# mkangquantum/quits

Hardware: AMD Instinct MI355X
Metric: decoded shots/sec + logical-error-rate, [[144,12,12]] BB code, d rounds, p=0.003 (higher is better)
Workload: dtype f32

## Files before the change

### quits_amd/csrc/bp_scatter_wide.hip

```cpp
#include "qd_internal.h"
#include "../../include/quits_amd.h"
#include "bp_scatter_edge.h"

#ifndef QSW_SCAT_SGPR_POS
#define QSW_SCAT_SGPR_POS 1
#endif
#ifndef QSW_GPRIO
#define QSW_GPRIO 1
#endif
#ifndef QSW_FAST_START
#define QSW_FAST_START 1
#endif
#ifndef QSW_THIN_LAST
#define QSW_THIN_LAST 1
#endif
#ifndef QSW_PRIO_BASE
#define QSW_PRIO_BASE 0
#endif

__device__ __forceinline__ uint4 qs_reuse4(uint4 &v) { asm volatile("" : "+v"(v.x), "+v"(v.y), "+v"(v.z), "+v"(v.w)); return v; }

template <int T, int MW, int CPL, int NSW>
__global__ void __launch_bounds__(T, MW) qd_bp_scatter_wide_kernel(BpGraphDev g, ScatGraphDev sg, DecodeArgs a, ScatArgs x)
{
// ... 310 lines not shown
            }
            return;
        }
    }
    for (int b = tid; b < sg.nslots; b += T)
        if (*QS_LDS(cur + 4u * (uint32_t)b) < 0) {
            const uint32_t jf = sg.slot_fault[b];
            if (jf != 0xFFFFFFFFu) atomicOr(&outw[jf >> 5], 1u << (jf & 31u));
        }
    if (!converged && a.want_llr && tid == 0) misc[48] = atomicAdd(a.fail_count, 1);
    __syncthreads();
    for (int w = tid; w < g.out_words; w += T) a.err_bits[shot * g.out_words + w] = outw[w];
    if (!converged && a.want_llr) {
        const int slot = misc[48];
        float *dst = a.llr_ws + (int64_t)slot * n_pad;
        for (int k1 = tid; k1 < g.n; k1 += T) dst[k1] = (float)(*QS_LDS(cur + 4u * sg.k1_slot[k1]) + 1) * x.grid_inv;
        if (tid == 0) a.fail_list[slot] = (int32_t)shot;
    }
    if (tid == 0) a.status[shot] = t | (converged << 16) | a.status_or;
}

#undef QS_ACC
#define QS_ACC(off) (prior_g[((uint32_t)(off) - (uint32_t)sg.offA) >> 2])
#define QS_ADJ(row_) qs_as_uint4(__builtin_amdgcn_raw_buffer_load_b128(adj_rsrc, adj_voff, (row_) * adj_row, 0))
#define QS_ABL_ADJC
template <int NSW>
__global__ void __launch_bounds__(64) qd_bp_first_pass_kernel(BpGraphDev g, ScatGraphDev sg, const int32_t *prior_g, uint32_t *rec)
{
    static_assert(NSW == 3, "the record has room for three sign words");
    const int c = (int)blockIdx.x * 64 + (int)threadIdx.x;
    const bool actv = c < g.m;
    constexpr int j = 0;
// ... 59 lines not shown
```

### quits_amd/csrc/osd_shared.h

```cpp
#pragma once
#include "qd_internal.h"

#define QD_NOKEY 0xFFFFFFFFu

#ifdef QD_OSD_TIMING
#define QD_TICK(slot)                                                                   \
    {                                                                                   \
        const unsigned long long now_ = wall_clock64();                                 \
        acc_[slot] += now_ - tick_;                                                     \
        tick_ = now_;                                                                   \
    }
#else
#define QD_TICK(slot)
#endif

__device__ __forceinline__ uint64_t &qd_qword(uint64_t *q_lds, uint64_t *q_glb, int kw_lds, int m_pad, int w, int r)
{
    return (w < kw_lds) ? q_lds[(size_t)w * m_pad + r] : q_glb[(size_t)(w - kw_lds) * m_pad + r];
}

__device__ __forceinline__ uint32_t qd_mono_key(float llr)
{
    const float f = llr + 0.0f;
    const uint32_t u = __float_as_uint(f);
    return (u & 0x80000000u) ? ~u : (u | 0x80000000u);
}

template <int T>
__device__ __forceinline__ void qd_bitonic_u64(uint64_t *buf, int P, int tid)
{
    for (int k = 2; k <= P; k <<= 1)
        for (int j = k >> 1; j > 0; j >>= 1) {
            for (int pi = tid; pi < (P >> 1); pi += T) {
                const int i = ((pi & ~(j - 1)) << 1) | (pi & (j - 1));
                const int l = i | j;
                const uint64_t x = buf[i], y = buf[l];
                const bool up = ((i & k) == 0);
                if ((x > y) == up) { buf[i] = y; buf[l] = x; }
            }
            __syncthreads();
        }
}

#define QD_OSD_TIER 1024
#ifndef QD_OSD_FULL_PAIRS
#define QD_OSD_FULL_PAIRS 1
#endif
#ifndef QD_OSD_TIER_FIRST
#define QD_OSD_TIER_FIRST 256
#endif
#define QD_OSD_KWR 6
#ifndef QD_OSD_KWR0
#define QD_OSD_KWR0 2
#endif
#ifndef QD_OSD_KPT
#define QD_OSD_KPT 1
#endif

template <int T>
__device__ __forceinline__ uint32_t qd_block_sum(uint32_t v, uint32_t *buf, int &phase)
{
    constexpr int NW = T / 64;
    v = qd_wave_add(v);
    if ((threadIdx.x & 63) == 0) buf[phase * 64 + (threadIdx.x >> 6)] = v;
// ... 19 lines not shown
    const uint8_t *det, *upd;
    int64_t det_stride, det_offset, upd_stride;
    const float *llr_ws;
    const int32_t *fail_list, *fail_count;
    const int32_t *slot_list, *slot_count;
    uint64_t *q_spill_fast;
    uint64_t *mt_ws;
    uint32_t *err_bits;
    int32_t *status;
    unsigned long long *dbg;
};

struct TierState {
    uint32_t lo_key, lo_idx; int sphase, exhausted, limit;
    uint32_t guess = 0u, cut = 0u, count = 0u;
};

#ifndef QD_OSD_TIER_INLINE
#define QD_OSD_TIER_INLINE __forceinline__
#endif
template <int T, int KPT = QD_OSD_KPT, class ARGS = OsdRegArgs, int SCAN = 0>
__device__ QD_OSD_TIER_INLINE int qd_osd_draw_tier(const ARGS &a, const float *llr, uint64_t *sortbuf, uint16_t *order,
                                             uint32_t *red, uint32_t *sumbuf, TierState &ts)
{
    const int tid = threadIdx.x;
    const int n = a.n;
    const bool in_regs = n <= KPT * T;
    uint32_t lo_key = ts.lo_key, lo_idx = ts.lo_idx;
    int sphase = ts.sphase;
    const uint32_t lim = (uint32_t)ts.limit;
    bool exhausted = false;
    int cnt = 0;
    {
            uint32_t kreg[KPT];
            if (in_regs) {
#pragma unroll
                for (int i = 0; i < KPT; ++i) {
                    const int b = tid + i * T;
                    kreg[i] = (b < n) ? qd_mono_key(llr[b]) : 0xFFFFFFFFu;
                }
            }
            auto scan_keys = [&](auto fn) {
                if constexpr (SCAN == 0) {
                    for (int b = tid; b < n; b += T) fn(qd_mono_key(llr[b]), b);
                } else {
                    const float4 *l4 = reinterpret_cast<const float4 *>(llr);
                    const int n4 = n >> 2;
                    for (int b0 = 0; b0 < n4; b0 += SCAN * T) {
// ... 137 lines not shown
                if (take) {
                    const uint32_t at = atomicAdd(&red[80], 1u);
                    if (at < (uint32_t)QD_OSD_TIER) sortbuf[at] = ((uint64_t)u << 32) | j;
                }
            });
            __syncthreads();
            if (!spec) break;
            {
                const uint32_t c = (uint32_t)__builtin_amdgcn_readfirstlane((int)red[80]);
                ts.count = c;
                if (c > 0u && c <= lim) { cnt = (int)c; lo_key = t_hi; ts.cut = t_hi; break; }
                spec = false;
                __syncthreads();
            }
            }
            int P = 64;
            while (P < cnt) P <<= 1;
            for (int i = cnt + tid; i < P; i += T) sortbuf[i] = ~0ull;
            __syncthreads();
            if (cnt <= 256 && cnt <= T) {
                if ((tid & ~63) < cnt) {
                    const uint64_t mine = tid < cnt ? sortbuf[tid] : ~0ull;
                    const uint4 *sb4 = reinterpret_cast<const uint4 *>(sortbuf);
                    int rank = 0;
                    for (int i = 0; i < (cnt + 1) / 2; ++i) {
                        const uint4 v = sb4[i];
                        const uint64_t k0 = (uint64_t)v.x | ((uint64_t)v.y << 32), k1 = (uint64_t)v.z | ((uint64_t)v.w << 32);
                        rank += (k0 < mine ? 1 : 0) + (k1 < mine ? 1 : 0);
                    }
                    if (tid < cnt) order[rank] = (uint16_t)(mine & 0xFFFFu);
                }
            } else {
                qd_bitonic_u64<T>(sortbuf, P, tid);
                for (int i = tid; i < cnt; i += T) order[i] = (uint16_t)(sortbuf[i] & 0xFFFFu);
            }
            __syncthreads();
    }
    ts.lo_key = lo_key; ts.lo_idx = lo_idx; ts.sphase = sphase; ts.exhausted = 0;
    return cnt;
}

struct OsdLds {
    uint64_t *q;
    uint64_t *tb;
    uint8_t *sp;
    int16_t *rowpiv;
    uint16_t *prow;
    uint32_t *pcol;
    uint32_t *pairs;
    uint32_t *bcols;
    uint32_t *red;
    uint32_t *outw;
// ... 177 lines not shown
```

### quits_amd/csrc/osd_sr.hip

```cpp
#include "osd_shared.h"
#include <algorithm>

#ifndef QD_SR_TIER_GUESS
#define QD_SR_TIER_GUESS 1
#endif
struct OsdSrArgs {
    int m, n, m_pad, n_pad, mw, out_words, upd_rows, ell_log2;
    int o_tb, o_rowpiv, o_prow, o_pcol, o_ppos, o_nz, o_cand, o_stq, o_stsp, o_bcols, o_red, o_out, o_order;
    int tier_first;
    const uint16_t *csc_ell;
    const uint32_t *bit_orig;
    const uint8_t *det, *upd;
    int64_t det_stride, det_offset, upd_stride;
    const float *llr_ws;
    const int32_t *fail_list, *fail_count;
    uint64_t *q_spill;
    int32_t *hard_list, *hard_count;
    uint32_t *err_bits;
    int32_t *status;
    unsigned long long *dbg;
};

template <int T, int RPT, int KWR>
__global__ void __launch_bounds__(T, QD_SR_WPS_OF(RPT)) qd_osd0_sr_kernel(OsdSrArgs a)
{
    extern __shared__ __align__(16) unsigned char smem[];
#if QD_SR_PRIO
    __builtin_amdgcn_s_setprio(QD_SR_PRIO);
#endif
    const int tid = threadIdx.x, lane = tid & 63;
    constexpr int NW = T / 64;
    static_assert(NW <= 16 && T >= 256, "key / flag records hold 16 wavefronts; the tier drawing wants >= 256 threads");
    uint64_t *tb = reinterpret_cast<uint64_t *>(smem + a.o_tb);
    uint64_t *sortbuf = tb;
    int16_t *rowpiv = reinterpret_cast<int16_t *>(smem + a.o_rowpiv);
    uint16_t *prow = reinterpret_cast<uint16_t *>(smem + a.o_prow);
    uint32_t *pcol = reinterpret_cast<uint32_t *>(smem + a.o_pcol);
    uint16_t *ppos = reinterpret_cast<uint16_t *>(smem + a.o_ppos);
    uint64_t *nz = reinterpret_cast<uint64_t *>(smem + a.o_nz);
    uint32_t *cand = reinterpret_cast<uint32_t *>(smem + a.o_cand);
    uint64_t *stq = reinterpret_cast<uint64_t *>(smem + a.o_stq);
    uint32_t *stsp = reinterpret_cast<uint32_t *>(smem + a.o_stsp);
    uint32_t *bcols = reinterpret_cast<uint32_t *>(smem + a.o_bcols);
    uint32_t *red = reinterpret_cast<uint32_t *>(smem + a.o_red);
    uint32_t *sumbuf = red + 96;
    uint32_t *outw = reinterpret_cast<uint32_t *>(smem + a.o_out);
    uint16_t *order = reinterpret_cast<uint16_t *>(smem + a.o_order);
    const int m = a.m, m_pad = a.m_pad, mw = a.mw, dlog = a.ell_log2;
    uint64_t *qglb = a.q_spill + (size_t)blockIdx.x * (size_t)(mw > KWR ? mw - KWR : 0) * m_pad;
    const int nfail = *a.fail_count;
    if (tid == 0) red[81] = 0u;
    for (int item = blockIdx.x; item < nfail; item += gridDim.x) {
        const int slot = item;
        const int64_t shot = a.fail_list[slot];
        const float *llr = a.llr_ws + (int64_t)slot * a.n_pad;
        const uint8_t *det = a.det + shot * a.det_stride + a.det_offset;
        const uint8_t *upd = a.upd ? a.upd + shot * a.upd_stride : nullptr;
#ifdef QD_OSD_TIMING
        unsigned long long acc_[12] = {0, 0, 0, 0, 0, 0, 0, 0, 0, 0, 0, 0};
        unsigned long long tick_ = wall_clock64();
#endif
        uint64_t my_tb[RPT], my_q[RPT][KWR];
        uint32_t my_sp = 0, my_piv = 0;
#pragma unroll
        for (int i = 0; i < RPT; ++i) {
            const int r = tid + i * T;
            uint32_t sbit = 0;
            if (r < m) {
                sbit = det[r] & 1u;
                if (upd && r < a.upd_rows) sbit ^= upd[r] & 1u;
            }
            my_sp |= sbit << i;
            my_tb[i] = 0ull;
#pragma unroll
            for (int w = 0; w < KWR; ++w) my_q[i][w] = 0ull;
            if (r < m_pad) rowpiv[r] = -1;
        }
        for (int w = tid; w < a.out_words; w += T) outw[w] = 0u;
        if (tid < 240) cand[tid] = (tid % 80) < 64 ? QD_NOKEY : 0u;
        if (tid == 0) red[72] = 0u;
        __syncthreads();
        QD_TICK(10)

        int npiv = 0, done = 0, draining = 0, cmaxp1 = 64, sphase = 0, rd = 0, bseq = 0, ntier = 0;
        uint32_t my_bp = 0;
        uint32_t lo_key = 0, lo_idx = 0;
        while (!done) {
            TierState ts{lo_key, lo_idx, sphase, 0, ntier == 0 ? a.tier_first : QD_OSD_TIER};
            const bool first_tier = ntier == 0;
            if (first_tier) ts.guess = red[81];
            ++ntier;
            const int cnt = qd_osd_draw_tier<T, QD_OSD_KPT, OsdSrArgs, 6>(a, llr, sortbuf, order, red, sumbuf, ts);
            lo_key = ts.lo_key; lo_idx = ts.lo_idx; sphase = ts.sphase;
            if (first_tier && QD_SR_TIER_GUESS) {
                const uint32_t lim1 = (uint32_t)a.tier_first, step = 1u << 20;
                uint32_t g = ts.guess;
                if (ts.cut) g = ts.count * 20u > lim1 * 17u ? ts.cut - step : (ts.count * 20u < lim1 * 11u ? ts.cut + step : ts.cut);
                else if (g) g = ts.count > lim1 ? g - step : g;
                if (g > 0xFFFFFFFFu - step) g = 0u;
                if (tid == 0) red[81] = g;
            }
            QD_TICK(0)
            if (ts.exhausted) break;
            for (int base = 0; base < cnt && !done; base += 64, ++bseq) {
                const int nb = min(64, cnt - base);
#pragma unroll
                for (int i = 0; i < RPT; ++i) { const int r = tid + i * T; if (r < m_pad) tb[r] = 0ull; }
                if (tid < mw) nz[tid] = 0ull;
                if (tid < 64) bcols[tid] = tid < nb ? (uint32_t)order[base + tid] : 0xFFFFFFFFu;
                __syncthreads();
                for (int x = tid; x < (64 << dlog); x += T) {
                    const int c = x >> dlog, q = x & ((1 << dlog) - 1);
                    const uint32_t col = bcols[c];
                    if (col != 0xFFFFFFFFu) {
                        const uint32_t r = a.csc_ell[((size_t)col << dlog) + q];
// ... 173 lines not shown
            if (draining && ((my_bp >> i) & 1u) && (int)(ppos[rowpiv[r]] & 63u) >= cmaxp1) ++over;
        }
        const uint32_t tot = qd_block_sum<T>(over | (resid << 16), sumbuf, sphase);
        const int inconsistent = (tot >> 16) != 0u;
        const int npiv_rep = npiv - (int)(tot & 0xFFFFu);
        if (inconsistent) {
            if (tid == 0) a.hard_list[atomicAdd(a.hard_count, 1)] = slot;
        } else {
#pragma unroll
            for (int i = 0; i < RPT; ++i)
                if (((my_piv >> i) & 1u) && ((my_sp >> i) & 1u)) {
                    const uint32_t j = pcol[rowpiv[tid + i * T]];
                    atomicOr(&outw[j >> 5], 1u << (j & 31u));
                }
            __syncthreads();
            for (int w = tid; w < a.out_words; w += T) a.err_bits[shot * a.out_words + w] = outw[w];
            if (tid == 0) a.status[shot] = (a.status[shot] & 0xFFFF) | (1 << 17) | (min(npiv_rep, 4095) << 20);
        }
        QD_TICK(3)
#ifdef QD_OSD_TIMING
        if (tid == 0) {
            for (int i = 0; i < 8; ++i) atomicAdd(&a.dbg[i], acc_[i]);
            atomicAdd(&a.dbg[8], 1ull); atomicAdd(&a.dbg[9], (unsigned long long)npiv); atomicAdd(&a.dbg[10], acc_[10]); atomicAdd(&a.dbg[11], acc_[11]); atomicAdd(&a.dbg[12], (unsigned long long)ntier); atomicAdd(&a.dbg[13], (unsigned long long)bseq);
        }
#endif
        __syncthreads();
    }
}

int qd_osd_sr_layout(int m, int m_pad, int n, int out_words, int *off13, int *threads, int *rpt)
{
    if (m > 2048 || n > 49152) return 0;
    const int T = m <= 256 ? 256 : (m <= 4 * QD_SR_TSMALL ? QD_SR_TSMALL : 512);
    *threads = T; *rpt = (m + T - 1) / T;
    auto al = [](int x) { return (x + 15) & ~15; };
    int o = 0;
    off13[0] = o; o += al(std::max(m_pad * 8, QD_OSD_TIER * 8));
    off13[1] = o; o += al(m_pad * 2);
    off13[2] = o; o += al(m_pad * 2);
    off13[3] = o; o += al(m_pad * 4);
    off13[4] = o; o += al(m_pad * 2);
    off13[5] = o; o += al(((m + 63) / 64) * 8);
    off13[6] = o; o += 3 * 80 * 4;
    off13[7] = o; o += (QD_SR_KWR_MAX + 1) * 64 * 8;
    off13[8] = o; o += 64 * 4;
    off13[9] = o; o += 64 * 4;
    off13[10] = o; o += 1024;
    off13[11] = o; o += al(out_words * 4);
    off13[12] = o; o += al(QD_OSD_TIER * 2);
    return o;
}

size_t qd_osd_sr_ws_words(int m_pad, int mw, int threads, int rpt)
{
    (void)threads;
    const int kwr = QD_SR_KWR_OF(rpt);
    return (size_t)(mw > kwr ? mw - kwr : 0) * m_pad + 64;
}

hipError_t qd_launch_osd0_sr(const OsdGraphDev &g, const BpGraphDev &bg, const DecodeArgs &a, int blocks, hipStream_t s)
{
    OsdSrArgs r{};
    r.m = g.m; r.n = g.n; r.m_pad = g.m_pad; r.n_pad = bg.n_pad; r.mw = g.mw; r.out_words = bg.out_words; r.upd_rows = a.upd_rows;
    r.ell_log2 = g.ell_log2;
    const int *o = g.s_off;
    r.o_tb = o[0]; r.o_rowpiv = o[1]; r.o_prow = o[2]; r.o_pcol = o[3]; r.o_ppos = o[4]; r.o_nz = o[5]; r.o_cand = o[6]; r.o_stq = o[7];
    r.o_stsp = o[8]; r.o_bcols = o[9]; r.o_red = o[10]; r.o_out = o[11]; r.o_order = o[12];
    r.tier_first = QD_OSD_TIER_FIRST;
    r.csc_ell = g.csc_ell; r.bit_orig = bg.bit_orig;
    r.det = a.det; r.upd = a.upd; r.det_stride = a.det_stride; r.det_offset = a.det_offset; r.upd_stride = a.upd_stride;
    r.llr_ws = a.llr_ws; r.fail_list = a.fail_list; r.fail_count = a.fail_count; r.q_spill = a.q_spill_sr;
    r.hard_list = a.hard_list; r.hard_count = a.hard_count;
    r.err_bits = a.err_bits; r.status = a.status; r.dbg = a.dbg;
    const int lds = g.s_lds_bytes;
#define QD_SR_CASE(TT, RR)                                                                                                        \
    {                                                                                                                             \
        auto k = qd_osd0_sr_kernel<TT, RR, QD_SR_KWR_OF(RR)>;                                                                            \
        hipError_t e = hipFuncSetAttribute((const void *)k, hipFuncAttributeMaxDynamicSharedMemorySize, lds);                     \
        if (e != hipSuccess) return e;                                                                                            \
        hipLaunchKernelGGL(k, dim3((unsigned)blocks), dim3(TT), lds, s, r);                                                       \
        return hipGetLastError();                                                                                                 \
    }
    if (g.s_threads == 256) {
        switch (g.s_rpt) {
        case 1: QD_SR_CASE(256, 1)
        case 2: QD_SR_CASE(256, 2)
        case 3: QD_SR_CASE(256, 3)
        default: QD_SR_CASE(256, 4)
// ... 11 lines not shown
```

### quits_amd/csrc/qd_api.hip

```cpp
#include "../../include/quits_amd.h"
#include "qd_internal.h"

#include <algorithm>
#include <cmath>
#include <cstdarg>
#include <cstdio>
#include <cstdlib>
#include <cstring>
#include <memory>
#include <numeric>
#include <vector>

#define QD_GEN_PREFIX_LDS (32 * 1024)

hipError_t qd_launch_bp(const BpGraphDev &g, const DecodeArgs &a, int64_t B, hipStream_t s);
hipError_t qd_launch_bp_scatter(const BpGraphDev &g, const ScatGraphDev &sg, const DecodeArgs &a, const ScatArgs &x, int64_t B, hipStream_t s);
hipError_t qd_launch_bp_scatter_wide(const BpGraphDev &g, const ScatGraphDev &sg, const DecodeArgs &a, const ScatArgs &x, int64_t B, hipStream_t s);
hipError_t qd_launch_bp_first_pass(const BpGraphDev &g, const ScatGraphDev &sg, const int32_t *prior_g, uint32_t *rec, hipStream_t s);
hipError_t qd_launch_bp_general(const GenGraphDev &g, const BpGraphDev &bg, const DecodeArgs &a, const GenWs &w, int bp_method,
                                int schedule, int64_t shot0, int nshots, hipStream_t s, GenStagePlan *plan);
hipError_t qd_launch_hold(const int32_t *count, int threshold, int microseconds, hipStream_t s);
int qd_bp_ps_lds_bytes(const GenGraphDev &g, int max_rdeg);
hipError_t qd_launch_bp_ps_lds(const GenGraphDev &g, const BpGraphDev &bg, const DecodeArgs &a, int64_t B, hipStream_t s);
hipError_t qd_launch_osd0(const OsdGraphDev &g, const BpGraphDev &bg, const DecodeArgs &a, int blocks_fast,
// ... 49 lines not shown
        size_t bytes = std::max<size_t>(h.size() * sizeof(Tp), 16);
        if (hipMalloc(&d, bytes) != hipSuccess) return -1;
        ptrs.push_back(d);
        if (!h.empty() && hipMemcpy(d, h.data(), h.size() * sizeof(Tp), hipMemcpyHostToDevice) != hipSuccess) return -1;
        *out = reinterpret_cast<const Tp *>(d);
        return 0;
    }
    void release()
    {
        for (void *p : ptrs) (void)hipFree(p);
        ptrs.clear();
    }
};

struct Switches {
    bool no_scatter, scatter_cpl1, scatter_wide_t704, scatter_natural_rounds, scatter_banks_by_slot, scatter_walk_greedy, osdcs_old, bp_no_fast_start;
    float scatter_m2_limit;
    std::vector<int> gen_stages;
};

static Switches read_switches()
{
    auto env = [](const char *name) { return std::getenv(name); };
    Switches w{};
    w.no_scatter = env("QD_NO_SCATTER") != nullptr;
    w.scatter_cpl1 = env("QD_SCATTER_CPL1") != nullptr;
    w.scatter_wide_t704 = env("QD_SCATTER_WIDE_T704") != nullptr;
    w.scatter_natural_rounds = env("QD_SCATTER_NATURAL_ROUNDS") != nullptr;
    w.scatter_banks_by_slot = env("QD_SCATTER_BANKS_BY_SLOT") != nullptr;
    w.scatter_walk_greedy = env("QD_SCATTER_WALK_GREEDY") != nullptr;
    const char *ev = env("QD_BP_NO_FAST_START");
    w.bp_no_fast_start = ev && std::atoi(ev) == 1;
    ev = env("QD_OSDCS_OLD");
    w.osdcs_old = ev && std::atoi(ev) == 1;
    ev = env("QD_SCATTER_M2_LIMIT");
    w.scatter_m2_limit = ev ? (float)std::atof(ev) : INFINITY;
    w.gen_stages = {3, 6, 10, 14, 20, 28, 40, 56, 80, 112};
    if ((ev = env("QD_GEN_STAGES"))) {
        w.gen_stages.clear();
        for (const char *q = ev; *q;) {
            char *end = nullptr;
            const long v = std::strtol(q, &end, 10);
            if (end == q) break;
            if (v > 0) w.gen_stages.push_back((int)v);
            q = *end ? end + 1 : end;
        }
    }
// ... 63 lines not shown
    GenStagePlan gsp{};
    int gen_bounds[QD_GEN_MAX_STAGES] = {0}, gen_nbounds = 0;
    int grid_k = -1, grid_kc = -1, grid_floor = 0;
    BpGraphDev bp_fine{}, bp_coarse{};
    const float *llr0_q = nullptr;
    const float *llr0_qc = nullptr;
    bool off_chip = false;
    bool edge_cert = false;
    int32_t *redo_list = nullptr;
    int redo_cap = 0;
    const int32_t *prior_g = nullptr;
    float m2_limit = 0.f;
    const uint32_t *first_pass = nullptr;
    int32_t *recheck_list = nullptr;
    int recheck_cap = 0;
    DevAllocs mem;
    int profiling = 0;
    struct Span { int kind; hipEvent_t t0, t1; };
    std::vector<Span> ev;
    double acc_ms[4] = {0, 0, 0, 0};
};

struct qd_spmat {
    int device = 0;
    SpmatDev d{};
    DevAllocs mem;
};

#define QD_GRID_MIN_BITS 10
static inline int align16(int x) { return (x + 15) & ~15; }
// ... 117 lines not shown
                int fb = 0;
                for (int l = 0; l < 32; ++l) {
                    const bool real_lane = l < gn;
                    const int deg = real_lane ? (int)(row_ptr[chk_orig[g0 + l] + 1] - row_ptr[chk_orig[g0 + l]]) : 0;
                    if (k < deg) continue;
                    while (fb < 32 && used[fb]) ++fb;
                    const int b = fb < 32 ? fb : (l & 31);
                    if (fb < 32) used[fb]++;
                    if (g0 + l < ((m + 63) & ~63)) put(g0 + l, k, -1, b);
                }
            }
        }
    }
}

extern "C" int qd_version(void) { return 107; }
extern "C" const char *qd_last_error(void) { return g_err; }
extern "C" int qd_device_count(void)
{
    int n = 0;
    if (hipGetDeviceCount(&n) != hipSuccess) return 0;
    return n;
}

struct HostGraph {
    int m = 0, n = 0, nnz = 0, max_rdeg = 0, max_cdeg = 0, min_rdeg = 0, m_pad = 0, n_pad = 0, max_rdeg_pad = 0;
    const int32_t *row_ptr = nullptr, *col_idx = nullptr;
    const double *priors = nullptr;
    std::vector<int> rdeg, cdeg;
    std::vector<double> llr0;
    std::vector<int32_t> cp, ri, pos;
// ... 708 lines not shown
            if (mxp < (1ll << 22) && lim > 0) {
                rc |= d->mem.upload(pg, &d->prior_g);
                d->m2_limit = std::min((float)lim, env.scatter_m2_limit);
                d->bp = g->sc.wide_threads ? BP_SCATTER_WIDE : BP_SCATTER;
                if (d->bp == BP_SCATTER_WIDE && !env.bp_no_fast_start && rc == 0) {
                    const std::vector<uint32_t> zero((size_t)g->bp.m_pad * 8, 0u);
                    rc |= d->mem.upload(zero, &d->first_pass);
                    if (rc == 0 && (qd_launch_bp_first_pass(d->bp_fine, g->sc, d->prior_g, const_cast<uint32_t *>(d->first_pass), nullptr) != hipSuccess ||
                                    hipStreamSynchronize(nullptr) != hipSuccess))
                        rc = -1;
                }
            }
        }
        if (rc) { d->mem.release(); delete d; return fail(QD_EHIP, "device allocation failed while building the LLR grid"); }
    }
    *out = d;
    return QD_OK;
}

extern "C" int qd_decoder_info(const qd_decoder *d, int32_t *info)
{
    if (!d || !info) return fail(QD_EINVAL, "null argument");
    info[0] = d->grid_k; info[1] = d->grid_kc; info[2] = d->bp == BP_LDS_EDGE || d->bp == BP_HBM_EDGE;
    info[3] = d->bp == BP_SCATTER_WIDE ? 2 : (d->bp == BP_SCATTER ? 1 : 0);
    return QD_OK;
}

extern "C" int qd_decoder_fast_start(const qd_decoder *d) { return d ? (d->first_pass != nullptr && d->prm.max_iter >= 1) : -1; }

extern "C" int qd_decoder_postproc_kernel(const qd_decoder *d) { return d ? d->post : -1; }

static void free_ws(qd_decoder *d)
{
    auto dev = [](auto *&p) { if (p) (void)hipFree(p); p = nullptr; };
    auto host = [](auto *&p) { if (p) (void)hipHostFree(p); p = nullptr; };
    auto event = [](hipEvent_t &e) { if (e) (void)hipEventDestroy(e); e = nullptr; };
    dev(d->llr_ws); dev(d->fail_list); dev(d->ctr_base); dev(d->order_ws); dev(d->q_spill); dev(d->q_spill_fast); dev(d->q_spill_sr); dev(d->q_spill_off);
    dev(d->mt_ws); dev(d->cs_ws); dev(d->hard_list); dev(d->hard_list2); dev(d->redo_list); dev(d->recheck_list); dev(d->lsd_ws);
    dev(d->gws.b2c); dev(d->gws.c2b); dev(d->gws.th); dev(d->gws.pre); dev(d->gws.llr); dev(d->gws.syn); dev(d->gws.slot);
    dev(d->gsp.msg2); dev(d->gsp.syn2); dev(d->gsp.lists[0]); dev(d->gsp.lists[1]); dev(d->gsp.counts);
    host(d->host_fail); host(d->gsp.host_counts);
    event(d->fail_ready); event(d->gsp.counts_ready);
    d->gws = GenWs{}; d->gsp = GenStagePlan{};
    d->fail_count = nullptr; d->fail_pending = false;
    d->post_blocks = d->redo_cap = d->recheck_cap = 0; d->cap = 0;
}

extern "C" void qd_decoder_destroy(qd_decoder *d)
{
    if (!d) return;
    (void)hipSetDevice(d->g->device);
    free_ws(d);
    d->mem.release();
// ... 39 lines not shown
        hipDeviceProp_t prop;
        if (hipGetDeviceProperties(&prop, g->device) == hipSuccess && prop.multiProcessorCount > 0) ncu = prop.multiProcessorCount;
        const int per_cu = std::max(1, QD_LDS_BYTES / std::max(1, g->osd.lds_bytes));
        d->osd_blocks = g->osd.lds_bytes > 0 ? ncu * std::min(per_cu, 2048 / std::max(1, g->osd.threads)) : 0;
        const int per_cu_fast = std::max(1, QD_LDS_BYTES / std::max(1, g->osd.f_lds_bytes));
        d->osd_blocks_fast = ncu * std::min(per_cu_fast, 2048 / std::max(1, g->osd.f_threads));
        if (d->osd_w) d->osd_blocks_fast = ncu;
        if (d->post == QD_POST_LSD) {
            const int lds = qd_lsd_lds_bytes(g->m, g->n, g->bp.out_words);
            d->post_blocks = ncu * std::max(1, std::min(8, QD_LDS_BYTES / std::max(1, lds)));
            HIP_TRY(hipMalloc((void **)&d->lsd_ws, qd_lsd_ws_bytes(g->m, g->n, d->post_blocks, d->lsd_w)));
        } else if (d->post == QD_POST_OSD0_SR) {
            d->post_blocks = ncu * g->osd.s_per_cu;
            HIP_TRY(hipMalloc((void **)&d->q_spill_sr, sizeof(uint64_t) * (size_t)d->post_blocks *
                                                       qd_osd_sr_ws_words(g->osd.m_pad, g->osd.mw, g->osd.s_threads, g->osd.s_rpt)));
        } else if (d->post == QD_POST_OSD_CS_PANEL) {
            d->post_blocks = ncu * d->cs_per_cu;
            HIP_TRY(hipMalloc((void **)&d->cs_ws, sizeof(uint64_t) * (size_t)d->post_blocks * qd_osdcs_ws_words(d->cs_variant)));
        }
        const int spill_fast = g->osd.mw - (d->osd_w ? g->osd.w_kw : g->osd.f_kw);
        if (g->osd.f_lds_bytes > 0 && spill_fast > 0)
            HIP_TRY(hipMalloc((void **)&d->q_spill_fast, sizeof(uint64_t) * (size_t)d->osd_blocks_fast * spill_fast * g->osd.m_pad));
        if (d->osd_w && g->osd.w_lds_bytes > 0)
            HIP_TRY(hipMalloc((void **)&d->mt_ws, sizeof(uint64_t) * (size_t)d->osd_blocks_fast * ((size_t)g->osd.mw * g->osd.m_pad + 64 * 32)));
        HIP_TRY(hipMalloc((void **)&d->hard_list, sizeof(int32_t) * (size_t)max_batch));
        HIP_TRY(hipMalloc((void **)&d->hard_list2, sizeof(int32_t) * (size_t)max_batch));
        HIP_TRY(hipMalloc((void **)&d->llr_ws, sizeof(float) * (size_t)max_batch * g->bp.n_pad));
        HIP_TRY(hipMalloc((void **)&d->fail_list, sizeof(int32_t) * (size_t)max_batch));
        if (d->osd_blocks > 0)
            HIP_TRY(hipMalloc((void **)&d->order_ws, sizeof(uint16_t) * (size_t)d->osd_blocks * g->n));
// ... 99 lines not shown
}

static DecodeArgs decode_args(const qd_decoder *d, const uint8_t *d_det, int64_t det_stride, int64_t det_offset, const uint8_t *d_upd,
                              int64_t upd_stride, int32_t upd_rows, uint32_t *d_err_bits, int32_t *d_status)
{
    DecodeArgs a{};
    a.det = d_det; a.det_stride = det_stride; a.det_offset = det_offset;
    a.upd = d_upd; a.upd_stride = upd_stride; a.upd_rows = d_upd ? upd_rows : 0;
    a.max_iter = d->prm.max_iter; a.ms_scale = (float)d->prm.ms_scaling_factor; a.want_llr = d->post != QD_POST_NONE ? 1 : 0;
    a.err_bits = d_err_bits; a.status = d_status;
    a.llr_ws = d->llr_ws; a.fail_list = d->fail_list; a.fail_count = d->fail_count;
    a.order_ws = d->order_ws; a.q_spill = d->q_spill; a.q_spill_fast = d->q_spill_fast; a.q_spill_sr = d->q_spill_sr; a.mt_ws = d->mt_ws;
    a.hard_list = d->hard_list; a.hard_list2 = d->hard_list2; a.hard_count = d->fail_count + 1;
    a.dbg = reinterpret_cast<unsigned long long *>(d->ctr_base) + 2;
    a.osd_w = d->osd_w; a.osd_order = d->prm.osd_order; a.rank = d->g->rank;
    return a;
}

static int launch_bp(qd_decoder *d, const DecodeArgs &a, int64_t B, hipStream_t s)
{
    const qd_graph *g = d->g;
    GenGraphDev gg = g->gen;
    gg.llr0 = d->llr0_q;
    switch (d->bp) {
    case BP_LDS_EDGE: HIP_TRY(qd_launch_bp_ps_lds(gg, g->bp, a, B, s)); break;
    case BP_GATHER_RAW: HIP_TRY(qd_launch_bp(g->bp, a, B, s)); break;
    case BP_HBM_EDGE: {
        int32_t *redo_count = d->fail_count + 40;
        DecodeArgs a1 = a;
        if (d->edge_cert) {
// ... 58 lines not shown
        HIP_TRY(qd_launch_lsd0(g->gen, g->bp, a, d->lsd_ws, d->post_blocks, blocks, d->lsd_w, d->prm.osd_order, g->osd.wfix, s));
        break;
    case QD_POST_OSD_CS_PANEL:
        HIP_TRY(qd_launch_osdcs(g->osd, g->bp, a, d->cs_off, d->cs_variant, d->cs_lds, d->cs_ws, blocks, s));
        break;
    case QD_POST_OSD0_SR:
        HIP_TRY(qd_launch_osd0_sr(g->osd, g->bp, a, blocks, s));
        HIP_TRY(qd_launch_osd0(g->osd, g->bp, a, fast, full, s, true));
        break;
    default:
        HIP_TRY(qd_launch_osd0(g->osd, g->bp, a, fast, full, s));
    }
    return QD_OK;
}

static int decode_impl(qd_decoder *d, const uint8_t *d_det, int64_t det_stride, int64_t det_offset, const uint8_t *d_upd,
                       int64_t upd_stride, int32_t upd_rows, int64_t B, uint32_t *d_err_bits, int32_t *d_status, int stage,
                       void *stream)
{
    if (!d) return fail(QD_EINVAL, "null decoder");
    if (stage < 1 || stage > 3) return fail(QD_EINVAL, "stage must be 1 (BP), 2 (OSD) or 3 (both)");
    if (int rc = check_batch(d, det_stride, det_offset, d_upd, upd_stride, upd_rows, B)) return rc;
    if (B == 0) return QD_OK;
    if (!d_det || !d_err_bits || !d_status) return fail(QD_EINVAL, "null argument");
    HIP_TRY(hipSetDevice(d->g->device));
    if (B > d->cap && stage == 2) return fail(QD_EINVAL, "OSD stage without a preceding BP stage of this batch size");
    if (int rc = B > d->cap ? qd_decoder_reserve(d, B) : QD_OK) return rc;
    hipStream_t s = reinterpret_cast<hipStream_t>(stream);
    const bool post = d->post != QD_POST_NONE;
    if (stage & 1) {
        d->cset ^= 1;
        d->fail_count = d->ctr_base + 64 * d->cset;
        if (!d->set_clean[d->cset]) {
            HIP_TRY(hipMemsetAsync(d->fail_count, 0, 3 * sizeof(int32_t), s));
            HIP_TRY(hipMemsetAsync(d->fail_count + 40, 0, 2 * sizeof(int32_t), s));
        }
        d->set_clean[d->cset] = false;
        d->last_B = B;
    }
    const DecodeArgs a = decode_args(d, d_det, det_stride, det_offset, d_upd, upd_stride, upd_rows, d_err_bits, d_status);
    auto span = [&](int kind) -> int {
        if (!d->profiling) return QD_OK;
        hipEvent_t t0, t1;
        HIP_TRY(hipEventCreate(&t0)); HIP_TRY(hipEventCreate(&t1));
        d->ev.push_back({kind, t0, t1});
        HIP_TRY(hipEventRecord(t0, s));
        return QD_OK;
    };
    if (stage & 1) {
        if (int rc = span(0)) return rc;
        if (int rc = launch_bp(d, a, B, s)) return rc;
        if (d->profiling) HIP_TRY(hipEventRecord(d->ev.back().t1, s));
    }
// ... 49 lines not shown
    return decode_impl(d, d_det, det_stride, det_offset, d_upd, upd_stride, upd_rows, B, d_err_bits, d_status, stage, stream);
}

extern "C" int qd_osd0_batch(qd_decoder *d, const uint8_t *d_det, int64_t det_stride, int64_t det_offset,
                             const uint8_t *d_upd, int64_t upd_stride, int32_t upd_rows, int64_t B, const float *d_llr,
                             uint32_t *d_err_bits, int32_t *d_status, void *stream)
{
    if (!d) return fail(QD_EINVAL, "null decoder");
    if (d->post == QD_POST_NONE) return fail(QD_EINVAL, "decoder was created with osd_method = off");
    if (int rc = check_batch(d, det_stride, det_offset, d_upd, upd_stride, upd_rows, B)) return rc;
    if (B == 0) return QD_OK;
    if (!d_det || !d_llr || !d_err_bits || !d_status) return fail(QD_EINVAL, "null argument");
    HIP_TRY(hipSetDevice(d->g->device));
    if (int rc = B > d->cap ? qd_decoder_reserve(d, B) : QD_OK) return rc;
    hipStream_t s = reinterpret_cast<hipStream_t>(stream);
    const DecodeArgs a = decode_args(d, d_det, det_stride, det_offset, d_upd, upd_stride, upd_rows, d_err_bits, d_status);
    HIP_TRY(hipMemsetAsync(d->fail_count, 0, 3 * sizeof(int32_t), s));
    d->set_clean[d->cset] = false;
    HIP_TRY(qd_launch_stage_llr(d_llr, d->g->n, d->g->bp.n_pad, d->g->bp.bit_orig, B, d->llr_ws, d->fail_list, d->fail_count,
                                d_status, s));
    return launch_post(d, a, B, s);
}

extern "C" int qd_decoder_debug_counters(qd_decoder *d, uint64_t *out16)
{
    if (!d || !out16 || !d->fail_count) return fail(QD_EINVAL, "no workspace yet");
    HIP_TRY(hipSetDevice(d->g->device));
    HIP_TRY(hipDeviceSynchronize());
    HIP_TRY(hipMemcpy(out16, reinterpret_cast<char *>(d->ctr_base) + 16, 16 * sizeof(uint64_t), hipMemcpyDeviceToHost));
    HIP_TRY(hipMemset(reinterpret_cast<char *>(d->ctr_base) + 16, 0, 16 * sizeof(uint64_t)));
// ... 262 lines not shown
```

### quits_amd/csrc/qd_internal.h

```cpp
#pragma once
#include <hip/hip_runtime.h>
#include <stdint.h>

#define QD_WAVE 64
#define QD_MAX_COL_DEG 16
#define QD_MAX_ROW_DEG 255
#define QD_LDS_BYTES (160 * 1024)
#ifndef QD_SR_KWR
#define QD_SR_KWR 4
#endif
#ifndef QD_SR_WPS12
#define QD_SR_WPS12 4
#endif
#ifndef QD_SR_KWR_OF
#define QD_SR_KWR_OF(rpt) QD_SR_KWR
#endif
#ifndef QD_SR_WPS_OF
#define QD_SR_WPS_OF(rpt) ((rpt) <= 2 ? QD_SR_WPS12 : 2)
#endif
#ifndef QD_SR_TSMALL
#define QD_SR_TSMALL 512
#endif
#define QD_SR_KWR_MAX (QD_SR_KWR > 4 ? QD_SR_KWR : 4)

struct BpGraphDev {
    int m, n, m_pad, n_pad;
    int max_rdeg, max_cdeg, neg_words, out_words;
    int max_rdeg_pad;
    int dummy_bit, dummy_chk;
    int rec_words;
    int sign_mode;
    int adj32;
    const void *chk_adj;
    const int32_t *chk_degp_w;
    const uint32_t *chk_orig;
    const uint32_t *bit_rec;
    const uint32_t *bit_orig;
    const uint32_t *bit_slot_of;
// ... 124 lines not shown
    uint64_t *q_spill_fast;
    uint64_t *q_spill_sr;
    uint64_t *mt_ws;
    int32_t *hard_list;
    int32_t *hard_list2;
    int32_t *hard_count;
    unsigned long long *dbg;
    int osd_w, osd_order, rank;
    float s_limit;
    const int32_t *shot_list;
    const int32_t *shot_count;
    int32_t *redo_list;
    int32_t *redo_count;
    int redo_cap;
    int status_or;
};

__device__ __forceinline__ int qd_block_or(int pred, int *red, int nwaves, int phase)
{
    const unsigned long long bal = __ballot(pred);
    if ((threadIdx.x & 63) == 0) red[phase * 16 + (threadIdx.x >> 6)] = (bal != 0ull);
    __syncthreads();
    const int4 *r4 = reinterpret_cast<const int4 *>(red + phase * 16);
    int r = 0;
    for (int w = 0; w < (nwaves + 3) / 4; ++w) {
        const int4 v = r4[w];
        r |= v.x | v.y | v.z | v.w;
    }
    return r;
}
// ... 66 lines not shown
```

Baseline: 1.579 million.

## Hand over first OSD tier from BP kernel to OSD stage

When BP fails to converge, the scatter-wide BP kernel now also picks the low-reliability bits whose key falls below a shared cut and writes them, with a header, into a per-slot tier workspace. The OSD-SR kernel reads that list and uses it as its first tier, so it no longer rescans all LLRs for that tier. Tier-cut guessing is extended to the second tier, and the shared cut is updated across kernels through a device word. Epoch tagging guards against stale lists. This adds global writes and atomics to the BP epilogue, plus a new workspace buffer, in exchange.

```diff
diff --git a/quits_amd/csrc/bp_scatter_wide.hip b/quits_amd/csrc/bp_scatter_wide.hip
--- a/quits_amd/csrc/bp_scatter_wide.hip
+++ b/quits_amd/csrc/bp_scatter_wide.hip
@@ -348,8 +348,22 @@
     if (!converged && a.want_llr) {
         const int slot = misc[48];
         float *dst = a.llr_ws + (int64_t)slot * n_pad;
-        for (int k1 = tid; k1 < g.n; k1 += T) dst[k1] = (float)(*QS_LDS(cur + 4u * sg.k1_slot[k1]) + 1) * x.grid_inv;
+        const uint32_t cutk = a.tier_ws ? __hip_atomic_load(QD_TIER_CUT_WORD(a.tier_ws), __ATOMIC_RELAXED, __HIP_MEMORY_SCOPE_AGENT) : 0u;
+        uint64_t *tl = a.tier_ws + (int64_t)slot * QD_TIER_ROW;
+        for (int k1 = tid; k1 < g.n; k1 += T) {
+            const float v = (float)(*QS_LDS(cur + 4u * sg.k1_slot[k1]) + 1) * x.grid_inv;
+            dst[k1] = v;
+            const uint32_t key = qd_mono_key(v);
+            if (key < cutk) {
+                const uint32_t at = (uint32_t)atomicAdd(&misc[49], 1);
+                if (at < (uint32_t)QD_OSD_TIER_FIRST) tl[2 + at] = ((uint64_t)key << 32) | g.bit_orig[k1];
+            }
+        }
         if (tid == 0) a.fail_list[slot] = (int32_t)shot;
+        if (a.tier_ws) {
+            __syncthreads();
+            if (tid == 0) *reinterpret_cast<uint4 *>(tl) = make_uint4((uint32_t)misc[49], cutk, (uint32_t)shot, a.tier_epoch);
+        }
     }
     if (tid == 0) a.status[shot] = t | (converged << 16) | a.status_or;
 }
diff --git a/quits_amd/csrc/osd_shared.h b/quits_amd/csrc/osd_shared.h
--- a/quits_amd/csrc/osd_shared.h
+++ b/quits_amd/csrc/osd_shared.h
@@ -19,12 +19,6 @@
     return (w < kw_lds) ? q_lds[(size_t)w * m_pad + r] : q_glb[(size_t)(w - kw_lds) * m_pad + r];
 }
 
-__device__ __forceinline__ uint32_t qd_mono_key(float llr)
-{
-    const float f = llr + 0.0f;
-    const uint32_t u = __float_as_uint(f);
-    return (u & 0x80000000u) ? ~u : (u | 0x80000000u);
-}
 
 template <int T>
 __device__ __forceinline__ void qd_bitonic_u64(uint64_t *buf, int P, int tid)
@@ -42,12 +36,36 @@
         }
 }
 
+template <int T>
+__device__ __forceinline__ void qd_osd_rank_tier(uint64_t *sortbuf, uint16_t *order, int cnt)
+{
+    const int tid = threadIdx.x;
+    int P = 64;
+    while (P < cnt) P <<= 1;
+    for (int i = cnt + tid; i < P; i += T) sortbuf[i] = ~0ull;
+    __syncthreads();
+    if (cnt <= 256 && cnt <= T) {
+        if ((tid & ~63) < cnt) {
+            const uint64_t mine = tid < cnt ? sortbuf[tid] : ~0ull;
+            const uint4 *sb4 = reinterpret_cast<const uint4 *>(sortbuf);
+            int rank = 0;
+            for (int i = 0; i < (cnt + 1) / 2; ++i) {
+                const uint4 v = sb4[i];
+                const uint64_t k0 = (uint64_t)v.x | ((uint64_t)v.y << 32), k1 = (uint64_t)v.z | ((uint64_t)v.w << 32);
+                rank += (k0 < mine ? 1 : 0) + (k1 < mine ? 1 : 0);
+            }
+            if (tid < cnt) order[rank] = (uint16_t)(mine & 0xFFFFu);
+        }
+    } else {
+        qd_bitonic_u64<T>(sortbuf, P, tid);
+        for (int i = tid; i < cnt; i += T) order[i] = (uint16_t)(sortbuf[i] & 0xFFFFu);
+    }
+    __syncthreads();
+}
+
 #define QD_OSD_TIER 1024
 #ifndef QD_OSD_FULL_PAIRS
 #define QD_OSD_FULL_PAIRS 1
-#endif
-#ifndef QD_OSD_TIER_FIRST
-#define QD_OSD_TIER_FIRST 256
 #endif
 #define QD_OSD_KWR 6
 #ifndef QD_OSD_KWR0
@@ -97,6 +115,7 @@
 struct TierState {
     uint32_t lo_key, lo_idx; int sphase, exhausted, limit;
     uint32_t guess = 0u, cut = 0u, count = 0u;
+    uint32_t list_count = 0u, list_cut = 0u;
 };
 
 #ifndef QD_OSD_TIER_INLINE
@@ -114,7 +133,11 @@
     const uint32_t lim = (uint32_t)ts.limit;
     bool exhausted = false;
     int cnt = 0;
-    {
+    if (ts.list_count) {
+        cnt = (int)ts.list_count;
+        lo_key = ts.list_cut; lo_idx = 0u;
+        ts.cut = ts.list_cut; ts.count = ts.list_count;
+    } else {
             uint32_t kreg[KPT];
             if (in_regs) {
 #pragma unroll
@@ -282,28 +305,8 @@
                 __syncthreads();
             }
             }
-            int P = 64;
-            while (P < cnt) P <<= 1;
-            for (int i = cnt + tid; i < P; i += T) sortbuf[i] = ~0ull;
-            __syncthreads();
-            if (cnt <= 256 && cnt <= T) {
-                if ((tid & ~63) < cnt) {
-                    const uint64_t mine = tid < cnt ? sortbuf[tid] : ~0ull;
-                    const uint4 *sb4 = reinterpret_cast<const uint4 *>(sortbuf);
-                    int rank = 0;
-                    for (int i = 0; i < (cnt + 1) / 2; ++i) {
-                        const uint4 v = sb4[i];
-                        const uint64_t k0 = (uint64_t)v.x | ((uint64_t)v.y << 32), k1 = (uint64_t)v.z | ((uint64_t)v.w << 32);
-                        rank += (k0 < mine ? 1 : 0) + (k1 < mine ? 1 : 0);
-                    }
-                    if (tid < cnt) order[rank] = (uint16_t)(mine & 0xFFFFu);
-                }
-            } else {
-                qd_bitonic_u64<T>(sortbuf, P, tid);
-                for (int i = tid; i < cnt; i += T) order[i] = (uint16_t)(sortbuf[i] & 0xFFFFu);
-            }
-            __syncthreads();
-    }
+    }
+    qd_osd_rank_tier<T>(sortbuf, order, cnt);
     ts.lo_key = lo_key; ts.lo_idx = lo_idx; ts.sphase = sphase; ts.exhausted = 0;
     return cnt;
 }
diff --git a/quits_amd/csrc/osd_sr.hip b/quits_amd/csrc/osd_sr.hip
--- a/quits_amd/csrc/osd_sr.hip
+++ b/quits_amd/csrc/osd_sr.hip
@@ -4,9 +4,14 @@
 #ifndef QD_SR_TIER_GUESS
 #define QD_SR_TIER_GUESS 1
 #endif
+#define QD_SR_CAND_BYTES (3 * 80 * 4)
+#define QD_SR_STQ_BYTES ((QD_SR_KWR_MAX + 1) * 64 * 8)
+#ifndef QD_SR_TIER2_AIM
+#define QD_SR_TIER2_AIM QD_OSD_TIER
+#endif
 struct OsdSrArgs {
     int m, n, m_pad, n_pad, mw, out_words, upd_rows, ell_log2;
-    int o_tb, o_rowpiv, o_prow, o_pcol, o_ppos, o_nz, o_cand, o_stq, o_stsp, o_bcols, o_red, o_out, o_order;
+    int o_tb, o_rowpiv, o_prow, o_pcol, o_ppos, o_nz, o_cand, o_out, o_order;
     int tier_first;
     const uint16_t *csc_ell;
     const uint32_t *bit_orig;
@@ -19,6 +24,8 @@
     uint32_t *err_bits;
     int32_t *status;
     unsigned long long *dbg;
+    uint64_t *tier_ws;
+    uint32_t tier_epoch;
 };
 
 template <int T, int RPT, int KWR>
@@ -39,23 +46,33 @@
     uint16_t *ppos = reinterpret_cast<uint16_t *>(smem + a.o_ppos);
     uint64_t *nz = reinterpret_cast<uint64_t *>(smem + a.o_nz);
     uint32_t *cand = reinterpret_cast<uint32_t *>(smem + a.o_cand);
-    uint64_t *stq = reinterpret_cast<uint64_t *>(smem + a.o_stq);
-    uint32_t *stsp = reinterpret_cast<uint32_t *>(smem + a.o_stsp);
-    uint32_t *bcols = reinterpret_cast<uint32_t *>(smem + a.o_bcols);
-    uint32_t *red = reinterpret_cast<uint32_t *>(smem + a.o_red);
+    uint64_t *stq = reinterpret_cast<uint64_t *>(smem + a.o_cand + QD_SR_CAND_BYTES);
+    uint32_t *stsp = reinterpret_cast<uint32_t *>(smem + a.o_cand + QD_SR_CAND_BYTES + QD_SR_STQ_BYTES);
+    uint32_t *bcols = reinterpret_cast<uint32_t *>(smem + a.o_cand + QD_SR_CAND_BYTES + QD_SR_STQ_BYTES + 256);
+    uint32_t *red = reinterpret_cast<uint32_t *>(smem + a.o_cand + QD_SR_CAND_BYTES + QD_SR_STQ_BYTES + 512);
     uint32_t *sumbuf = red + 96;
     uint32_t *outw = reinterpret_cast<uint32_t *>(smem + a.o_out);
     uint16_t *order = reinterpret_cast<uint16_t *>(smem + a.o_order);
     const int m = a.m, m_pad = a.m_pad, mw = a.mw, dlog = a.ell_log2;
     uint64_t *qglb = a.q_spill + (size_t)blockIdx.x * (size_t)(mw > KWR ? mw - KWR : 0) * m_pad;
     const int nfail = *a.fail_count;
-    if (tid == 0) red[81] = 0u;
+    if (tid == 0) {
+        red[81] = a.tier_ws ? __hip_atomic_load(QD_TIER_CUT_WORD(a.tier_ws), __ATOMIC_RELAXED, __HIP_MEMORY_SCOPE_AGENT) : 0u;
+        red[82] = 0u;
+    }
     for (int item = blockIdx.x; item < nfail; item += gridDim.x) {
         const int slot = item;
         const int64_t shot = a.fail_list[slot];
         const float *llr = a.llr_ws + (int64_t)slot * a.n_pad;
         const uint8_t *det = a.det + shot * a.det_stride + a.det_offset;
         const uint8_t *upd = a.upd ? a.upd + shot * a.upd_stride : nullptr;
+        uint64_t tl_entry = 0ull;
+        uint4 tl_head = make_uint4(0u, 0u, 0u, 0u);
+        if (a.tier_ws) {
+            const uint64_t *tl = a.tier_ws + (int64_t)slot * QD_TIER_ROW;
+            tl_head = *reinterpret_cast<const uint4 *>(tl);
+            if (tid < QD_OSD_TIER_FIRST) tl_entry = tl[2 + tid];
+        }
 #ifdef QD_OSD_TIMING
         unsigned long long acc_[12] = {0, 0, 0, 0, 0, 0, 0, 0, 0, 0, 0, 0};
         unsigned long long tick_ = wall_clock64();
@@ -76,9 +93,14 @@
             for (int w = 0; w < KWR; ++w) my_q[i][w] = 0ull;
             if (r < m_pad) rowpiv[r] = -1;
         }
+#pragma unroll 1
         for (int w = tid; w < a.out_words; w += T) outw[w] = 0u;
         if (tid < 240) cand[tid] = (tid % 80) < 64 ? QD_NOKEY : 0u;
         if (tid == 0) red[72] = 0u;
+        if (a.tier_ws) {
+            if (tid < QD_OSD_TIER_FIRST) sortbuf[tid] = tl_entry;
+            if (tid == 0) *reinterpret_cast<uint4 *>(red + 84) = tl_head;
+        }
         __syncthreads();
         QD_TICK(10)
 
@@ -87,18 +109,33 @@
         uint32_t lo_key = 0, lo_idx = 0;
         while (!done) {
             TierState ts{lo_key, lo_idx, sphase, 0, ntier == 0 ? a.tier_first : QD_OSD_TIER};
-            const bool first_tier = ntier == 0;
-            if (first_tier) ts.guess = red[81];
+            const bool first_tier = ntier == 0, guessed = ntier <= 1 && QD_SR_TIER_GUESS;
+            if (ntier == 1) ts.guess = red[82];
+            if (first_tier) {
+                ts.guess = red[81];
+                if (a.tier_ws) {
+                    const uint4 h = *reinterpret_cast<const uint4 *>(red + 84);
+                    const uint32_t hc = (uint32_t)__builtin_amdgcn_readfirstlane((int)h.x), hk = (uint32_t)__builtin_amdgcn_readfirstlane((int)h.y);
+                    if ((uint32_t)__builtin_amdgcn_readfirstlane((int)h.z) == (uint32_t)shot && (uint32_t)__builtin_amdgcn_readfirstlane((int)h.w) == a.tier_epoch) {
+                        if (hc >= 1u && hc <= (uint32_t)QD_OSD_TIER_FIRST) { ts.list_count = hc; ts.list_cut = hk; }
+                        else if (hc == 0u ? ts.guess <= hk : ts.guess >= hk)
+                            ts.guess = 0u;
+                    }
+                }
+            }
             ++ntier;
             const int cnt = qd_osd_draw_tier<T, QD_OSD_KPT, OsdSrArgs, 6>(a, llr, sortbuf, order, red, sumbuf, ts);
             lo_key = ts.lo_key; lo_idx = ts.lo_idx; sphase = ts.sphase;
-            if (first_tier && QD_SR_TIER_GUESS) {
-                const uint32_t lim1 = (uint32_t)a.tier_first, step = 1u << 20;
+            if (guessed) {
+                const uint32_t lim1 = first_tier ? (uint32_t)a.tier_first : (uint32_t)QD_SR_TIER2_AIM, step = 1u << 20;
                 uint32_t g = ts.guess;
                 if (ts.cut) g = ts.count * 20u > lim1 * 17u ? ts.cut - step : (ts.count * 20u < lim1 * 11u ? ts.cut + step : ts.cut);
                 else if (g) g = ts.count > lim1 ? g - step : g;
                 if (g > 0xFFFFFFFFu - step) g = 0u;
-                if (tid == 0) red[81] = g;
+                if (tid == 0 && !(first_tier && (a.tier_epoch & QD_TIER_CUT_FIXED)) && g != red[first_tier ? 81 : 82]) {
+                    red[first_tier ? 81 : 82] = g;
+                    if (first_tier && a.tier_ws && blockIdx.x == 0) __hip_atomic_store(QD_TIER_CUT_WORD(a.tier_ws), g, __ATOMIC_RELAXED, __HIP_MEMORY_SCOPE_AGENT);
+                }
             }
             QD_TICK(0)
             if (ts.exhausted) break;
@@ -302,6 +339,7 @@
                     atomicOr(&outw[j >> 5], 1u << (j & 31u));
                 }
             __syncthreads();
+#pragma unroll 1
             for (int w = tid; w < a.out_words; w += T) a.err_bits[shot * a.out_words + w] = outw[w];
             if (tid == 0) a.status[shot] = (a.status[shot] & 0xFFFF) | (1 << 17) | (min(npiv_rep, 4095) << 20);
         }
@@ -329,8 +367,8 @@
     off13[3] = o; o += al(m_pad * 4);
     off13[4] = o; o += al(m_pad * 2);
     off13[5] = o; o += al(((m + 63) / 64) * 8);
-    off13[6] = o; o += 3 * 80 * 4;
-    off13[7] = o; o += (QD_SR_KWR_MAX + 1) * 64 * 8;
+    off13[6] = o; o += QD_SR_CAND_BYTES;
+    off13[7] = o; o += QD_SR_STQ_BYTES;
     off13[8] = o; o += 64 * 4;
     off13[9] = o; o += 64 * 4;
     off13[10] = o; o += 1024;
@@ -352,14 +390,16 @@
     r.m = g.m; r.n = g.n; r.m_pad = g.m_pad; r.n_pad = bg.n_pad; r.mw = g.mw; r.out_words = bg.out_words; r.upd_rows = a.upd_rows;
     r.ell_log2 = g.ell_log2;
     const int *o = g.s_off;
-    r.o_tb = o[0]; r.o_rowpiv = o[1]; r.o_prow = o[2]; r.o_pcol = o[3]; r.o_ppos = o[4]; r.o_nz = o[5]; r.o_cand = o[6]; r.o_stq = o[7];
-    r.o_stsp = o[8]; r.o_bcols = o[9]; r.o_red = o[10]; r.o_out = o[11]; r.o_order = o[12];
+    r.o_tb = o[0]; r.o_rowpiv = o[1]; r.o_prow = o[2]; r.o_pcol = o[3]; r.o_ppos = o[4]; r.o_nz = o[5]; r.o_cand = o[6];
+    r.o_out = o[11]; r.o_order = o[12];
+    if (o[7] != o[6] + QD_SR_CAND_BYTES || o[8] != o[7] + QD_SR_STQ_BYTES || o[9] != o[8] + 256 || o[10] != o[9] + 256) return hipErrorInvalidValue;
     r.tier_first = QD_OSD_TIER_FIRST;
     r.csc_ell = g.csc_ell; r.bit_orig = bg.bit_orig;
     r.det = a.det; r.upd = a.upd; r.det_stride = a.det_stride; r.det_offset = a.det_offset; r.upd_stride = a.upd_stride;
     r.llr_ws = a.llr_ws; r.fail_list = a.fail_list; r.fail_count = a.fail_count; r.q_spill = a.q_spill_sr;
     r.hard_list = a.hard_list; r.hard_count = a.hard_count;
     r.err_bits = a.err_bits; r.status = a.status; r.dbg = a.dbg;
+    r.tier_ws = a.tier_ws; r.tier_epoch = a.tier_epoch;
     const int lds = g.s_lds_bytes;
 #define QD_SR_CASE(TT, RR)                                                                                                        \
     {                                                                                                                             \
diff --git a/quits_amd/csrc/qd_api.hip b/quits_amd/csrc/qd_api.hip
--- a/quits_amd/csrc/qd_api.hip
+++ b/quits_amd/csrc/qd_api.hip
@@ -87,7 +87,8 @@
 };
 
 struct Switches {
-    bool no_scatter, scatter_cpl1, scatter_wide_t704, scatter_natural_rounds, scatter_banks_by_slot, scatter_walk_greedy, osdcs_old, bp_no_fast_start;
+    bool no_scatter, scatter_cpl1, scatter_wide_t704, scatter_natural_rounds, scatter_banks_by_slot, scatter_walk_greedy, osdcs_old, bp_no_fast_start, osd0_own_tier;
+    uint32_t osd0_tier_cut;
     float scatter_m2_limit;
     std::vector<int> gen_stages;
 };
@@ -104,6 +105,10 @@
     w.scatter_walk_greedy = env("QD_SCATTER_WALK_GREEDY") != nullptr;
     const char *ev = env("QD_BP_NO_FAST_START");
     w.bp_no_fast_start = ev && std::atoi(ev) == 1;
+    ev = env("QD_OSD0_OWN_TIER");
+    w.osd0_own_tier = ev && std::atoi(ev) == 1;
+    ev = env("QD_OSD0_TIER_CUT");
+    w.osd0_tier_cut = ev ? (uint32_t)std::strtoul(ev, nullptr, 0) : 0u;
     ev = env("QD_OSDCS_OLD");
     w.osdcs_old = ev && std::atoi(ev) == 1;
     ev = env("QD_SCATTER_M2_LIMIT");
@@ -197,6 +202,10 @@
     const uint32_t *first_pass = nullptr;
     int32_t *recheck_list = nullptr;
     int recheck_cap = 0;
+    uint64_t *tier_base = nullptr, *tier_ws = nullptr;
+    bool tier_handover = false;
+    uint32_t tier_cut_fixed = 0;
+    uint32_t tier_epoch = 0;
     DevAllocs mem;
     int profiling = 0;
     struct Span { int kind; hipEvent_t t0, t1; };
@@ -344,7 +353,7 @@
     }
 }
 
-extern "C" int qd_version(void) { return 107; }
+extern "C" int qd_version(void) { return 108; }
 extern "C" const char *qd_last_error(void) { return g_err; }
 extern "C" int qd_device_count(void)
 {
@@ -1083,6 +1092,7 @@
         }
         if (rc) { d->mem.release(); delete d; return fail(QD_EHIP, "device allocation failed while building the LLR grid"); }
     }
+    if (d->bp == BP_SCATTER_WIDE && d->post == QD_POST_OSD0_SR && !env.osd0_own_tier) { d->tier_handover = true; d->tier_cut_fixed = env.osd0_tier_cut; }
     *out = d;
     return QD_OK;
 }
@@ -1105,7 +1115,7 @@
     auto host = [](auto *&p) { if (p) (void)hipHostFree(p); p = nullptr; };
     auto event = [](hipEvent_t &e) { if (e) (void)hipEventDestroy(e); e = nullptr; };
     dev(d->llr_ws); dev(d->fail_list); dev(d->ctr_base); dev(d->order_ws); dev(d->q_spill); dev(d->q_spill_fast); dev(d->q_spill_sr); dev(d->q_spill_off);
-    dev(d->mt_ws); dev(d->cs_ws); dev(d->hard_list); dev(d->hard_list2); dev(d->redo_list); dev(d->recheck_list); dev(d->lsd_ws);
+    dev(d->tier_base); d->tier_ws = nullptr; dev(d->mt_ws); dev(d->cs_ws); dev(d->hard_list); dev(d->hard_list2); dev(d->redo_list); dev(d->recheck_list); dev(d->lsd_ws);
     dev(d->gws.b2c); dev(d->gws.c2b); dev(d->gws.th); dev(d->gws.pre); dev(d->gws.llr); dev(d->gws.syn); dev(d->gws.slot);
     dev(d->gsp.msg2); dev(d->gsp.syn2); dev(d->gsp.lists[0]); dev(d->gsp.lists[1]); dev(d->gsp.counts);
     host(d->host_fail); host(d->gsp.host_counts);
@@ -1175,6 +1185,12 @@
             d->post_blocks = ncu * g->osd.s_per_cu;
             HIP_TRY(hipMalloc((void **)&d->q_spill_sr, sizeof(uint64_t) * (size_t)d->post_blocks *
                                                        qd_osd_sr_ws_words(g->osd.m_pad, g->osd.mw, g->osd.s_threads, g->osd.s_rpt)));
+            if (d->tier_handover) {
+                HIP_TRY(hipMalloc((void **)&d->tier_base, sizeof(uint64_t) * ((size_t)max_batch * QD_TIER_ROW + 2)));
+                HIP_TRY(hipMemset(d->tier_base, 0, sizeof(uint64_t) * ((size_t)max_batch * QD_TIER_ROW + 2)));
+                d->tier_ws = d->tier_base + 2;
+                HIP_TRY(hipMemcpy(QD_TIER_CUT_WORD(d->tier_ws), &d->tier_cut_fixed, sizeof(uint32_t), hipMemcpyHostToDevice));
+            }
         } else if (d->post == QD_POST_OSD_CS_PANEL) {
             d->post_blocks = ncu * d->cs_per_cu;
             HIP_TRY(hipMalloc((void **)&d->cs_ws, sizeof(uint64_t) * (size_t)d->post_blocks * qd_osdcs_ws_words(d->cs_variant)));
@@ -1304,6 +1320,7 @@
     a.hard_list = d->hard_list; a.hard_list2 = d->hard_list2; a.hard_count = d->fail_count + 1;
     a.dbg = reinterpret_cast<unsigned long long *>(d->ctr_base) + 2;
     a.osd_w = d->osd_w; a.osd_order = d->prm.osd_order; a.rank = d->g->rank;
+    a.tier_ws = d->tier_ws; a.tier_epoch = d->tier_epoch | (d->tier_cut_fixed ? QD_TIER_CUT_FIXED : 0u);
     return a;
 }
 
@@ -1392,6 +1409,16 @@
     return QD_OK;
 }
 
+static int next_tier_epoch(qd_decoder *d, hipStream_t s)
+{
+    if (!d->tier_ws) return QD_OK;
+    if (++d->tier_epoch >= QD_TIER_CUT_FIXED) {
+        HIP_TRY(hipMemsetAsync(d->tier_ws, 0, sizeof(uint64_t) * (size_t)d->cap * QD_TIER_ROW, s));
+        d->tier_epoch = 1u;
+    }
+    return QD_OK;
+}
+
 static int decode_impl(qd_decoder *d, const uint8_t *d_det, int64_t det_stride, int64_t det_offset, const uint8_t *d_upd,
                        int64_t upd_stride, int32_t upd_rows, int64_t B, uint32_t *d_err_bits, int32_t *d_status, int stage,
                        void *stream)
@@ -1415,6 +1442,7 @@
         }
         d->set_clean[d->cset] = false;
         d->last_B = B;
+        if (int rc = next_tier_epoch(d, s)) return rc;
     }
     const DecodeArgs a = decode_args(d, d_det, det_stride, det_offset, d_upd, upd_stride, upd_rows, d_err_bits, d_status);
     auto span = [&](int kind) -> int {
@@ -1494,6 +1522,7 @@
     HIP_TRY(hipSetDevice(d->g->device));
     if (int rc = B > d->cap ? qd_decoder_reserve(d, B) : QD_OK) return rc;
     hipStream_t s = reinterpret_cast<hipStream_t>(stream);
+    if (int rc = next_tier_epoch(d, s)) return rc;
     const DecodeArgs a = decode_args(d, d_det, det_stride, det_offset, d_upd, upd_stride, upd_rows, d_err_bits, d_status);
     HIP_TRY(hipMemsetAsync(d->fail_count, 0, 3 * sizeof(int32_t), s));
     d->set_clean[d->cset] = false;
diff --git a/quits_amd/csrc/qd_internal.h b/quits_amd/csrc/qd_internal.h
--- a/quits_amd/csrc/qd_internal.h
+++ b/quits_amd/csrc/qd_internal.h
@@ -22,6 +22,19 @@
 #define QD_SR_TSMALL 512
 #endif
 #define QD_SR_KWR_MAX (QD_SR_KWR > 4 ? QD_SR_KWR : 4)
+#ifndef QD_OSD_TIER_FIRST
+#define QD_OSD_TIER_FIRST 256
+#endif
+#define QD_TIER_ROW (QD_OSD_TIER_FIRST + 2)
+#define QD_TIER_CUT_WORD(tier_ws) (reinterpret_cast<uint32_t *>(tier_ws) - 4)
+#define QD_TIER_CUT_FIXED 0x80000000u
+
+__device__ __forceinline__ uint32_t qd_mono_key(float llr)
+{
+    const float f = llr + 0.0f;
+    const uint32_t u = __float_as_uint(f);
+    return (u & 0x80000000u) ? ~u : (u | 0x80000000u);
+}
 
 struct BpGraphDev {
     int m, n, m_pad, n_pad;
@@ -176,6 +189,8 @@
     int32_t *redo_count;
     int redo_cap;
     int status_or;
+    uint64_t *tier_ws;
+    uint32_t tier_epoch;
 };
 
 __device__ __forceinline__ int qd_block_or(int pred, int *red, int nwaves, int phase)
```

Result: no change. 1.590 million (median of 6 runs) (+0.7%).
